# harmoniqs/Piccolo.jl

Hardware: AMD Instinct MI355X
Metric: constraint+Jacobian evals/sec, 3-transmon d=27 unitary, T=100 knots (higher is better)
Workload: dtype f64

## Files before the change

piccolo.jl_amd/csrc/pcl_device_common.hpp:

```cpp
#pragma once

#define PCL_DBG_WG 1024
#define PCL_DBG_WORDS (64 + 2 * PCL_DBG_WG)

#define PCL_NSP 8

typedef double double4_t __attribute__((ext_vector_type(4)));
typedef double double2_t __attribute__((ext_vector_type(2)));

struct KParams {
    const double *Z;
    const double *mu;
    double *delta;
    double *jac;
    double *hess;
    const double *G0;
    const int *upos;
    const double *ucoef;
    const int *csr_ptr;
    const int *csr_col;
    const double *csr_val;
    const int *csc_ptr;
    const int *csc_row;
    const double *csc_val;
    const int *x_offs;
    int x_off0;
    const int *umap;
    const double *ell_val;
    const int *ell_col;
    int ell_w, ell_lds;
    const unsigned char *uell_l;
    const double *uell_v;
    int uell_w;
    const double *ellt_val;
    const int *ellt_col;
    int ellt_w;
    const double *ug0;
    double *hpart;
    unsigned int *hcnt;
    int prof;
    long long *dbg;
    int ncw;
    int tab_lds;
    int contig;
    int all_matrix;
    int n_stream;
    int iso;
    long long z_batch_stride;
    long long g0_batch_stride;
    long long jac_per;
    long long hess_per;
    int n_upos;
    int d, n, m, K, z_dim, u_off, dt_off, batch;
    int cols;
    int nc;
    int S;
    int LD;
    int compact;
    int nt;
    double *expm;
    double *xout;
    int q;
    int lds_doubles;
    double pc[6];
    double *mpart;
    const double *mlam;
    int tail_mode;
    int v4_np;
    int v4_flags;
    unsigned int *tick;
    int tick_cpi;
    int tick_G;
    int tick_ahead;
    int *err;
};

template <bool TRANS_A>
__device__ __forceinline__ void mfma_gemm_lds(const double *__restrict__ A, int lda, const double *__restrict__ B,
                                              int ldb, double *__restrict__ C, int ldc, int M, int Nc, int Kd,
                                              int wave, int nwaves, int lane) {
    const int rt_n = (M + 15) >> 4, ct_n = (Nc + 15) >> 4, ks_n = (Kd + 3) >> 2;
    const int nt = rt_n * ct_n;
    const int li = lane & 15, lk = lane >> 4;
    for (int t0 = wave * 2; t0 < nt; t0 += nwaves * 2) {
        const int t1 = t0 + 1;
        const bool has1 = t1 < nt;
        const int rt0 = t0 % rt_n, ct0 = t0 / rt_n;
        const int rt1 = has1 ? t1 % rt_n : rt0, ct1 = has1 ? t1 / rt_n : ct0;
        const int row0 = rt0 * 16 + li, col0 = ct0 * 16 + li;
        const int row1 = rt1 * 16 + li, col1 = ct1 * 16 + li;
        const bool r0 = row0 < M, c0 = col0 < Nc, r1 = has1 && row1 < M, c1 = has1 && col1 < Nc;
        double4_t acc0 = {0.0, 0.0, 0.0, 0.0}, acc1 = {0.0, 0.0, 0.0, 0.0};
        for (int ks = 0; ks < ks_n; ++ks) {
            const int k = ks * 4 + lk;
            const bool kok = k < Kd;
            double a0 = 0.0, b0 = 0.0, a1 = 0.0, b1 = 0.0;
            if (r0 && kok) a0 = TRANS_A ? A[k + lda * row0] : A[row0 + lda * k];
            if (c0 && kok) b0 = B[k + ldb * col0];
            if (r1 && kok) a1 = TRANS_A ? A[k + lda * row1] : A[row1 + lda * k];
            if (c1 && kok) b1 = B[k + ldb * col1];
            acc0 = __builtin_amdgcn_mfma_f64_16x16x4f64(a0, b0, acc0, 0, 0, 0);
            acc1 = __builtin_amdgcn_mfma_f64_16x16x4f64(a1, b1, acc1, 0, 0, 0);
        }
        if (c0) {
#pragma unroll
            for (int r = 0; r < 4; ++r) {
                const int rr = rt0 * 16 + lk + 4 * r;
                if (rr < M) C[rr + ldc * col0] = acc0[r];
            }
        }
        if (c1) {
#pragma unroll
            for (int r = 0; r < 4; ++r) {
                const int rr = rt1 * 16 + lk + 4 * r;
                if (rr < M) C[rr + ldc * col1] = acc1[r];
            }
        }
    }
}

template <bool TRANS_A, bool ACC>
__device__ __forceinline__ void mfma_gemm_lds_acc(const double *__restrict__ A, int lda, const double *__restrict__ B, int ldb,
                                                  double *__restrict__ C, int ldc, int M, int Nc, int Kd, double alpha, int wave,
                                                  int nwaves, int lane) {
    const int rt_n = (M + 15) >> 4, ct_n = (Nc + 15) >> 4, ks_n = (Kd + 3) >> 2;
    const int nt = rt_n * ct_n;
    const int li = lane & 15, lk = lane >> 4;
    for (int t0 = wave * 2; t0 < nt; t0 += nwaves * 2) {
        const int t1 = t0 + 1;
        const bool has1 = t1 < nt;
        const int rt0 = t0 % rt_n, ct0 = t0 / rt_n;
        const int rt1 = has1 ? t1 % rt_n : rt0, ct1 = has1 ? t1 / rt_n : ct0;
        const int row0 = rt0 * 16 + li, col0 = ct0 * 16 + li;
        const int row1 = rt1 * 16 + li, col1 = ct1 * 16 + li;
        const bool r0 = row0 < M, c0 = col0 < Nc, r1 = has1 && row1 < M, c1 = has1 && col1 < Nc;
        double4_t acc0 = {0.0, 0.0, 0.0, 0.0}, acc1 = {0.0, 0.0, 0.0, 0.0};
        if (ACC) {
#pragma unroll
            for (int r = 0; r < 4; ++r) {
                const int rr0 = rt0 * 16 + lk + 4 * r, rr1 = rt1 * 16 + lk + 4 * r;
                if (c0 && rr0 < M) acc0[r] = C[rr0 + ldc * col0];
                if (c1 && rr1 < M) acc1[r] = C[rr1 + ldc * col1];
            }
        }
        for (int ks = 0; ks < ks_n; ks += 4) {
            double a0[4], b0[4], a1[4], b1[4];
#pragma unroll
            for (int u = 0; u < 4; ++u) {
                const int k = (ks + u) * 4 + lk;
                const bool kok = k < Kd;
                const bool pa0 = r0 && kok, pb0 = c0 && kok, pa1 = r1 && kok, pb1 = c1 && kok;
                const double va0 = A[pa0 ? (TRANS_A ? k + lda * row0 : row0 + lda * k) : 0], vb0 = B[pb0 ? k + ldb * col0 : 0];
                const double va1 = A[pa1 ? (TRANS_A ? k + lda * row1 : row1 + lda * k) : 0], vb1 = B[pb1 ? k + ldb * col1 : 0];
                a0[u] = pa0 ? alpha * va0 : 0.0;
                b0[u] = pb0 ? vb0 : 0.0;
                a1[u] = pa1 ? alpha * va1 : 0.0;
                b1[u] = pb1 ? vb1 : 0.0;
            }
#pragma unroll
            for (int u = 0; u < 4; ++u)
                if (ks + u < ks_n) {
                    acc0 = __builtin_amdgcn_mfma_f64_16x16x4f64(a0[u], b0[u], acc0, 0, 0, 0);
                    acc1 = __builtin_amdgcn_mfma_f64_16x16x4f64(a1[u], b1[u], acc1, 0, 0, 0);
                }
        }
        if (c0) {
#pragma unroll
            for (int r = 0; r < 4; ++r) {
                const int rr = rt0 * 16 + lk + 4 * r;
                if (rr < M) C[rr + ldc * col0] = acc0[r];
            }
        }
        if (c1) {
#pragma unroll
            for (int r = 0; r < 4; ++r) {
                const int rr = rt1 * 16 + lk + 4 * r;
                if (rr < M) C[rr + ldc * col1] = acc1[r];
            }
        }
    }
}
template <bool TRANS_A, bool ACC>
__device__ __forceinline__ void gemm_lds_acc(const double *A, int lda, const double *B, int ldb, double *C, int ldc, int M, int Nc, int Kd,
                                             double alpha) {
    mfma_gemm_lds_acc<TRANS_A, ACC>(A, lda, B, ldb, C, ldc, M, Nc, Kd, alpha, threadIdx.x >> 6, blockDim.x >> 6, threadIdx.x & 63);
}

template <bool TRANS_A>
__device__ __forceinline__ void valu_gemm_lds(const double *__restrict__ A, int lda, const double *__restrict__ B,
                                              int ldb, double *__restrict__ C, int ldc, int M, int Nc, int Kd,
                                              int tid, int nthreads) {
    for (int e = tid; e < M * Nc; e += nthreads) {
        const int i = e % M, j = e / M;
        double s = 0.0;
        for (int k = 0; k < Kd; ++k) s = fma(TRANS_A ? A[k + lda * i] : A[i + lda * k], B[k + ldb * j], s);
        C[i + ldc * j] = s;
    }
}

template <bool MFMA, bool TRANS_A>
__device__ __forceinline__ void gemm_lds(const double *A, int lda, const double *B, int ldb, double *C, int ldc, int M,
                                         int Nc, int Kd) {
    if (MFMA)
        mfma_gemm_lds<TRANS_A>(A, lda, B, ldb, C, ldc, M, Nc, Kd, threadIdx.x >> 6, blockDim.x >> 6,
                               threadIdx.x & 63);
    else
        valu_gemm_lds<TRANS_A>(A, lda, B, ldb, C, ldc, M, Nc, Kd, threadIdx.x, blockDim.x);
}

__device__ __forceinline__ void store2(double *p, double a, double b, int nt) {
    double2_t v = {a, b};
    if (nt == 2)
        asm volatile("global_store_dwordx4 %0, %1, off sc0 sc1" ::"v"(p), "v"(v) : "memory");
    else if (nt)
        __builtin_nontemporal_store(v, reinterpret_cast<double2_t *>(p));
    else
        *reinterpret_cast<double2_t *>(p) = v;
}

__device__ __forceinline__ void bpm_entry(double id, double c1, double c2, double g, double h2, double &mbp, double &bm) {
    const double e = __builtin_fma(c2, h2, id);
    mbp = -__builtin_fma(c1, g, e);
    bm = __builtin_fma(-c1, g, e);
}

template <int NT, bool TRANSPOSE = false>
__device__ __forceinline__ void load_tile(const double *__restrict__ src, double *__restrict__ dst, int n, int LD, int tid) {
    const int nn = n * n;
    for (int e0 = tid; e0 < nn; e0 += NT * 8) {
        double v[8];
#pragma unroll
        for (int j = 0; j < 8; ++j) v[j] = e0 + NT * j < nn ? src[e0 + NT * j] : 0.0;
#pragma unroll
        for (int j = 0; j < 8; ++j) {
            const int e = e0 + NT * j;
            if (e < nn) dst[TRANSPOSE ? (e / n) + LD * (e % n) : (e % n) + LD * (e / n)] = v[j];
        }
    }
}

__device__ __forceinline__ void build_G(const KParams &p, const double *__restrict__ G0, const double *__restrict__ zk,
                                        double *__restrict__ G, double *__restrict__ us) {
    const int n = p.n, LD = p.LD;
    for (int e = threadIdx.x; e < n * n; e += blockDim.x) G[(e % n) + LD * (e / n)] = G0[e];
    if ((int)threadIdx.x < p.m) us[threadIdx.x] = zk[p.u_off + threadIdx.x];
    __syncthreads();
    for (int q = threadIdx.x; q < p.n_upos; q += blockDim.x) {
        const int pos = p.upos[q];
        const int idx = (pos % n) + LD * (pos / n);
        double g = G[idx];
        for (int l = 0; l < p.m; ++l) g += us[l] * p.ucoef[(long long)q * p.m + l];
        G[idx] = g;
    }
}

__device__ __forceinline__ void wave_lds_sync() {
    asm volatile("s_waitcnt lgkmcnt(0)" ::: "memory");
    __builtin_amdgcn_wave_barrier();
}

#define PCL_MAXRT 4
#define PCL_MREG 8
#define PCL_PFC 4
#define PCL_PFW 2

__device__ __forceinline__ double wave_sum(double v) {
    for (int off = 32; off > 0; off >>= 1) v += __shfl_down(v, off, 64);
    return v;
}

template <int CTRL>
__device__ __forceinline__ double dpp_f64(double v) {
    int lo = __double2loint(v), hi = __double2hiint(v);
    lo = __builtin_amdgcn_update_dpp(lo, lo, CTRL, 0xf, 0xf, false);
    hi = __builtin_amdgcn_update_dpp(hi, hi, CTRL, 0xf, 0xf, false);
    return __hiloint2double(hi, lo);
}
__device__ __forceinline__ double row16_sum(double v) {
    v += dpp_f64<0xB1>(v);
    v += dpp_f64<0x4E>(v);
    v += dpp_f64<0x141>(v);
    v += dpp_f64<0x140>(v);
    return v;
}
```

piccolo.jl_amd/csrc/pcl_kernel_exp.hpp:

```cpp
#pragma once

#define PCL_EXP_COMPACT 1
#define PCL_EXP_MERIT 2

template <bool JAC, int MODE = 0>
__global__ __launch_bounds__(512) void pcl_exp_kernel(const KParams p, const double *__restrict__ Gjd, const int gl_lds) {
    extern __shared__ double lds[];
    constexpr bool COMPACT = JAC && (MODE & PCL_EXP_COMPACT), MERIT = JAC && (MODE & PCL_EXP_MERIT);
    const int n = p.n, LD = p.LD, nn = n * n, cols = p.cols;
    const int tid = threadIdx.x, nth = blockDim.x;
    const int ml = JAC ? max(p.m, 1) : 1;
    const int l = blockIdx.x % ml;
    const long long bk = blockIdx.x / ml;
    const int k = (int)(bk % p.K), b = (int)(bk / p.K);
    const bool fre = JAC && p.m > 0;
    const int tile = LD * n;
    double *A = lds, *T = A + tile, *S = T + tile;
    double *X = JAC ? S + tile : nullptr;
    double *Gl = (fre && gl_lds) ? X + tile : nullptr;
    double *XK = lds + ((JAC ? 4 : 3) + (Gl ? 1 : 0)) * tile;
    double *us = XK + LD * cols, *red = us + 32;
    const double *zk = p.Z + (long long)b * p.z_batch_stride + (long long)k * p.z_dim;
    const double *G0 = p.G0 + (long long)b * p.g0_batch_stride;
    const double *Gv = fre ? Gjd + (long long)l * nn : nullptr;
    const double h = zk[p.dt_off];
    build_G(p, G0, zk, A, us);
    __syncthreads();
    if (tid < 64) {
        double cs = 0.0;
        if (tid < n)
            for (int i = 0; i < n; ++i) cs += fabs(A[i + LD * tid]);
        red[tid] = cs;
    }
    __syncthreads();
    double nrm = 0.0;
    for (int j = 0; j < n; ++j) nrm = fmax(nrm, red[j]);
    double theta = fabs(h) * nrm;
    int sq = 0;
    while (theta > 0.25 && sq < 60) {
        theta *= 0.5;
        ++sq;
    }
    const double hs = ldexp(h, -sq);
    for (int e = tid; e < nn; e += nth) {
        const int idx = (e % n) + LD * (e / n);
        T[idx] = (e % n == e / n) ? 1.0 : 0.0;
        if (fre) X[idx] = 0.0;
        if (Gl) Gl[idx] = Gv[e];
    }
    __syncthreads();
    for (int j = 14; j >= 1; --j) {
        const double f = hs / j;
        if (fre) {
            gemm_lds<true, false>(A, LD, X, LD, S, LD, n, n, n);
            __syncthreads();
            if (Gl)
                gemm_lds<true, false>(Gl, LD, T, LD, X, LD, n, n, n);
            else
                gemm_lds<true, false>(Gv, n, T, LD, X, LD, n, n, n);
            __syncthreads();
            for (int e = tid; e < nn; e += nth) {
                const int idx = (e % n) + LD * (e / n);
                S[idx] = f * (S[idx] + X[idx]);
            }
            double *t = X;
            X = S;
            S = t;
            __syncthreads();
        }
        gemm_lds<true, false>(A, LD, T, LD, S, LD, n, n, n);
        __syncthreads();
        for (int e = tid; e < nn; e += nth) {
            const int idx = (e % n) + LD * (e / n);
            T[idx] = ((e % n == e / n) ? 1.0 : 0.0) + f * S[idx];
        }
        __syncthreads();
    }
    for (int i = 0; i < sq; ++i) {
        if (fre) {
            gemm_lds<true, false>(T, LD, X, LD, S, LD, n, n, n);
            gemm_lds<true, false>(X, LD, T, LD, A, LD, n, n, n);
            __syncthreads();
            for (int e = tid; e < nn; e += nth) {
                const int idx = (e % n) + LD * (e / n);
                X[idx] = S[idx] + A[idx];
            }
            __syncthreads();
        }
        gemm_lds<true, false>(T, LD, T, LD, S, LD, n, n, n);
        __syncthreads();
        double *t = T;
        T = S;
        S = t;
    }
    const int xo = p.x_off0 >= 0 ? p.x_off0 : p.x_offs[b];
    const int ne = n * cols;
    for (int e = tid; e < ne; e += nth) XK[(e % n) + LD * (e / n)] = zk[xo + e];
    __syncthreads();
    double *jv = JAC ? p.jac + bk * p.jac_per : nullptr;
    const int ncopy = COMPACT ? 1 : cols;
    const long long seg1 = (long long)ncopy * nn, tail0 = seg1 + (COMPACT ? 0 : ne);
    const int tw = (p.m + 1) * n;
    const double *lam = MERIT && p.mlam ? p.mlam + bk * ne : nullptr;
    double *part = MERIT ? p.mpart + bk * (p.m + 2) : nullptr;
    if (fre) {
        gemm_lds<true, false>(X, LD, XK, LD, S, LD, n, cols, n);
        if (MERIT && !lam) gemm_lds<true, false>(T, LD, XK, LD, A, LD, n, cols, n);
        __syncthreads();
        for (int e = tid; e < ne; e += nth) jv[tail0 + (long long)(e / n) * tw + l * n + (e % n)] = -S[(e % n) + LD * (e / n)];
        if (MERIT) {
            double v = 0.0;
            for (int e = tid; e < ne; e += nth) {
                const int idx = (e % n) + LD * (e / n);
                v = fma(lam ? lam[e] : zk[p.z_dim + xo + e] - A[idx], -S[idx], v);
            }
            v = exph_block_sum(v, red);
            if (tid == 0) part[l] = v;
        }
        __syncthreads();
    }
    if (l == 0) {
        gemm_lds<true, false>(T, LD, XK, LD, S, LD, n, cols, n);
        __syncthreads();
        if (p.delta) {
            double *dl = p.delta + bk * ne;
            for (int e = tid; e < ne; e += nth) dl[e] = zk[p.z_dim + xo + e] - S[(e % n) + LD * (e / n)];
        }
        if (JAC) {
            if (fre && (sq > 0 || (MERIT && !lam))) {
                build_G(p, G0, zk, A, us);
                __syncthreads();
            }
            gemm_lds<true, false>(A, LD, S, LD, X, LD, n, cols, n);
            __syncthreads();
            for (int e = tid; e < ne; e += nth) {
                jv[tail0 + (long long)(e / n) * tw + p.m * n + (e % n)] = -X[(e % n) + LD * (e / n)];
                if (!COMPACT) jv[seg1 + e] = 1.0;
            }
            if (MERIT) {
                double vh = 0.0, vp = 0.0;
                for (int e = tid; e < ne; e += nth) {
                    const int idx = (e % n) + LD * (e / n);
                    const double dl = zk[p.z_dim + xo + e] - S[idx], lm = lam ? lam[e] : dl;
                    vh = fma(lm, -X[idx], vh);
                    vp = fma(lm, dl, vp);
                }
                vh = exph_block_sum(vh, red);
                vp = exph_block_sum(vp, red);
                if (tid == 0) {
                    part[p.m] = vh;
                    part[p.m + 1] = lam ? vp : 0.5 * vp;
                }
            }
        }
    }
    if (JAC) {
        if (!(n & 1) && !((unsigned long long)jv & 15ull)) {
            const int half = nn >> 1;
            for (int c = l; c < ncopy; c += ml) {
                double *dst = jv + (long long)c * nn;
                for (int e2 = tid; e2 < half; e2 += nth) {
                    const int e = 2 * e2, idx = (e % n) + LD * (e / n);
                    const double2_t v = {-T[idx], -T[idx + 1]};
                    *reinterpret_cast<double2_t *>(dst + e) = v;
                }
            }
        } else {
            for (int c = l; c < ncopy; c += ml) {
                double *dst = jv + (long long)c * nn;
                for (int e = tid; e < nn; e += nth) dst[e] = -T[(e % n) + LD * (e / n)];
            }
        }
    }
}
```

Before: 40960.

## Restructure MFMA f64 GEMM tiles with double-buffered loads and shared operand pairs

Replaces both MFMA LDS GEMM paths with one templated tile-pair routine. It double-buffers operand loads (P/Q slots with sched_barrier) so LDS reads overlap MFMA issue, and reuses the A or B fragment when the two tiles a wave handles share a row or column block. It also peels the K tail out of the main loop and removes per-iteration bounds predicates. Separately, the elementwise loops in the expm kernel now step row and column indices incrementally instead of computing e%n and e/n each iteration. This adds code complexity and template instantiations, and may raise register pressure.

```diff
diff --git a/piccolo.jl_amd/csrc/pcl_device_common.hpp b/piccolo.jl_amd/csrc/pcl_device_common.hpp
--- a/piccolo.jl_amd/csrc/pcl_device_common.hpp
+++ b/piccolo.jl_amd/csrc/pcl_device_common.hpp
@@ -75,110 +75,169 @@
     int *err;
 };
 
-template <bool TRANS_A>
+#ifndef PCL_GEMM_U
+#define PCL_GEMM_U 1
+#endif
+enum { PCL_PAIR_GENERAL = 0, PCL_PAIR_SHARED_B = 1, PCL_PAIR_SHARED_A = 2, PCL_PAIR_SINGLE = 3 };
+
+template <bool TRANS_A, bool ACC, bool SCALED, int U, int MODE>
+__device__ __forceinline__ void mfma_tile_pair(const double *__restrict__ A, int lda, const double *__restrict__ B, int ldb,
+                                               double *__restrict__ C, int ldc, int M, int Nc, int Kd, double alpha, int rt0, int ct0,
+                                               int rt1, int ct1, int li, int lk) {
+    constexpr bool PAIR = MODE != PCL_PAIR_SINGLE;
+    constexpr bool A1 = MODE == PCL_PAIR_GENERAL || MODE == PCL_PAIR_SHARED_B;
+    constexpr bool B1 = MODE == PCL_PAIR_GENERAL || MODE == PCL_PAIR_SHARED_A;
+    const int row0 = rt0 * 16 + li, col0 = ct0 * 16 + li, row1 = rt1 * 16 + li, col1 = ct1 * 16 + li;
+    const bool c0 = col0 < Nc, c1 = PAIR && col1 < Nc;
+    const int rc0 = row0 < M ? row0 : 0, cc0 = c0 ? col0 : 0, rc1 = row1 < M ? row1 : 0, cc1 = c1 ? col1 : 0;
+    const int oa0 = TRANS_A ? lk + lda * rc0 : rc0 + lda * lk, oa1 = TRANS_A ? lk + lda * rc1 : rc1 + lda * lk;
+    const int ob0 = lk + ldb * cc0, ob1 = lk + ldb * cc1;
+    const int sa = TRANS_A ? 4 : 4 * lda;
+    const int ks_full = Kd >> 2;
+    double4_t acc0 = {0.0, 0.0, 0.0, 0.0}, acc1 = {0.0, 0.0, 0.0, 0.0};
+    struct Slots {
+        double a0[U], b0[U], a1[U], b1[U];
+    } P, Q;
+    auto load = [&](Slots &s, int u, int ks) {
+        const double va0 = A[oa0 + sa * ks];
+        s.a0[u] = SCALED ? alpha * va0 : va0;
+        s.b0[u] = B[ob0 + 4 * ks];
+        if (A1) {
+            const double va1 = A[oa1 + sa * ks];
+            s.a1[u] = SCALED ? alpha * va1 : va1;
+        }
+        if (B1) s.b1[u] = B[ob1 + 4 * ks];
+    };
+    auto product = [&](double x0, double y0, double x1, double y1) {
+        acc0 = __builtin_amdgcn_mfma_f64_16x16x4f64(x0, y0, acc0, 0, 0, 0);
+        if (PAIR) acc1 = __builtin_amdgcn_mfma_f64_16x16x4f64(A1 ? x1 : x0, B1 ? y1 : y0, acc1, 0, 0, 0);
+    };
+    const bool tail = (Kd & 3) != 0;
+    double ta0 = 0.0, tb0 = 0.0, ta1 = 0.0, tb1 = 0.0;
+    if (tail) {
+        const bool kok = ks_full * 4 + lk < Kd;
+        const double va0 = A[kok ? oa0 + sa * ks_full : 0], vb0 = B[kok ? ob0 + 4 * ks_full : 0];
+        ta0 = kok ? (SCALED ? alpha * va0 : va0) : 0.0;
+        tb0 = kok ? vb0 : 0.0;
+        if (A1) {
+            const double va1 = A[kok ? oa1 + sa * ks_full : 0];
+            ta1 = kok ? (SCALED ? alpha * va1 : va1) : 0.0;
+        }
+        if (B1) {
+            const double vb1 = B[kok ? ob1 + 4 * ks_full : 0];
+            tb1 = kok ? vb1 : 0.0;
+        }
+    }
+    if (ACC) {
+#pragma unroll
+        for (int r = 0; r < 4; ++r) {
+            const int rr0 = rt0 * 16 + lk + 4 * r, rr1 = rt1 * 16 + lk + 4 * r;
+            if (c0 && rr0 < M) acc0[r] = C[rr0 + ldc * col0];
+            if (c1 && rr1 < M) acc1[r] = C[rr1 + ldc * col1];
+        }
+    }
+    auto request_whole = [&](Slots &s, int ks) {
+#pragma unroll
+        for (int u = 0; u < U; ++u) load(s, u, ks + u);
+    };
+    auto request = [&](Slots &s, int ks) {
+#pragma unroll
+        for (int u = 0; u < U; ++u) load(s, u, ks + u < ks_full ? ks + u : ks_full - 1);
+    };
+    auto spend_whole = [&](const Slots &s) {
+#pragma unroll
+        for (int u = 0; u < U; ++u) product(s.a0[u], s.b0[u], s.a1[u], s.b1[u]);
+    };
+    auto spend = [&](const Slots &s, int nb) {
+        if (nb >= U) {
+            spend_whole(s);
+        } else {
+#pragma unroll
+            for (int u = 0; u < U; ++u)
+                if (u < nb) product(s.a0[u], s.b0[u], s.a1[u], s.b1[u]);
+        }
+    };
+    if (ks_full > 0) {
+        int ks = 0;
+        request(P, 0);
+        for (; ks + 3 * U <= ks_full; ks += 2 * U) {
+            request_whole(Q, ks + U);
+            __builtin_amdgcn_sched_barrier(0x6);
+            spend_whole(P);
+            __builtin_amdgcn_sched_barrier(0x6);
+            request_whole(P, ks + 2 * U);
+            __builtin_amdgcn_sched_barrier(0x6);
+            spend_whole(Q);
+            __builtin_amdgcn_sched_barrier(0x6);
+        }
+        const int left = ks_full - ks;
+        if (left > U) request(Q, ks + U);
+        __builtin_amdgcn_sched_barrier(0x6);
+        spend(P, left);
+        if (left > U) {
+            __builtin_amdgcn_sched_barrier(0x6);
+            if (left > 2 * U) request(P, ks + 2 * U);
+            __builtin_amdgcn_sched_barrier(0x6);
+            spend(Q, left - U);
+            if (left > 2 * U) spend(P, left - 2 * U);
+        }
+    }
+    if (tail) product(ta0, tb0, ta1, tb1);
+    if (c0) {
+#pragma unroll
+        for (int r = 0; r < 4; ++r) {
+            const int rr = rt0 * 16 + lk + 4 * r;
+            if (rr < M) C[rr + ldc * col0] = acc0[r];
+        }
+    }
+    if (c1) {
+#pragma unroll
+        for (int r = 0; r < 4; ++r) {
+            const int rr = rt1 * 16 + lk + 4 * r;
+            if (rr < M) C[rr + ldc * col1] = acc1[r];
+        }
+    }
+}
+
+template <bool TRANS_A, bool ACC, bool SCALED, int U>
+__device__ __forceinline__ void mfma_gemm_tiles(const double *__restrict__ A, int lda, const double *__restrict__ B, int ldb,
+                                                double *__restrict__ C, int ldc, int M, int Nc, int Kd, double alpha, int wave,
+                                                int nwaves, int lane) {
+    const int rt_n = (M + 15) >> 4, ct_n = (Nc + 15) >> 4;
+    const int li = lane & 15, lk = lane >> 4;
+    const int step = 2 * nwaves;
+    int rt0 = 2 * __builtin_amdgcn_readfirstlane(wave), ct0 = 0;
+    if (rt_n <= 0) return;
+    for (;; rt0 += step) {
+        while (rt0 >= rt_n) rt0 -= rt_n, ++ct0;
+        if (ct0 >= ct_n) break;
+        const bool wrap = rt0 + 1 == rt_n;
+        const int rt1 = wrap ? 0 : rt0 + 1, ct1 = wrap ? ct0 + 1 : ct0;
+#define PCL_TILE_PAIR(MODE) mfma_tile_pair<TRANS_A, ACC, SCALED, U, MODE>(A, lda, B, ldb, C, ldc, M, Nc, Kd, alpha, rt0, ct0, rt1, ct1, li, lk)
+        if (ct1 >= ct_n)
+            PCL_TILE_PAIR(PCL_PAIR_SINGLE);
+        else if (!wrap)
+            PCL_TILE_PAIR(PCL_PAIR_SHARED_B);
+        else if (rt_n == 1)
+            PCL_TILE_PAIR(PCL_PAIR_SHARED_A);
+        else
+            mfma_tile_pair<TRANS_A, ACC, SCALED, (U > 1 ? U / 2 : 1), PCL_PAIR_GENERAL>(A, lda, B, ldb, C, ldc, M, Nc, Kd, alpha, rt0, ct0, rt1, ct1, li, lk);
+#undef PCL_TILE_PAIR
+    }
+}
+
+template <bool TRANS_A, int U = PCL_GEMM_U>
 __device__ __forceinline__ void mfma_gemm_lds(const double *__restrict__ A, int lda, const double *__restrict__ B,
                                               int ldb, double *__restrict__ C, int ldc, int M, int Nc, int Kd,
                                               int wave, int nwaves, int lane) {
-    const int rt_n = (M + 15) >> 4, ct_n = (Nc + 15) >> 4, ks_n = (Kd + 3) >> 2;
-    const int nt = rt_n * ct_n;
-    const int li = lane & 15, lk = lane >> 4;
-    for (int t0 = wave * 2; t0 < nt; t0 += nwaves * 2) {
-        const int t1 = t0 + 1;
-        const bool has1 = t1 < nt;
-        const int rt0 = t0 % rt_n, ct0 = t0 / rt_n;
-        const int rt1 = has1 ? t1 % rt_n : rt0, ct1 = has1 ? t1 / rt_n : ct0;
-        const int row0 = rt0 * 16 + li, col0 = ct0 * 16 + li;
-        const int row1 = rt1 * 16 + li, col1 = ct1 * 16 + li;
-        const bool r0 = row0 < M, c0 = col0 < Nc, r1 = has1 && row1 < M, c1 = has1 && col1 < Nc;
-        double4_t acc0 = {0.0, 0.0, 0.0, 0.0}, acc1 = {0.0, 0.0, 0.0, 0.0};
-        for (int ks = 0; ks < ks_n; ++ks) {
-            const int k = ks * 4 + lk;
-            const bool kok = k < Kd;
-            double a0 = 0.0, b0 = 0.0, a1 = 0.0, b1 = 0.0;
-            if (r0 && kok) a0 = TRANS_A ? A[k + lda * row0] : A[row0 + lda * k];
-            if (c0 && kok) b0 = B[k + ldb * col0];
-            if (r1 && kok) a1 = TRANS_A ? A[k + lda * row1] : A[row1 + lda * k];
-            if (c1 && kok) b1 = B[k + ldb * col1];
-            acc0 = __builtin_amdgcn_mfma_f64_16x16x4f64(a0, b0, acc0, 0, 0, 0);
-            acc1 = __builtin_amdgcn_mfma_f64_16x16x4f64(a1, b1, acc1, 0, 0, 0);
-        }
-        if (c0) {
-#pragma unroll
-            for (int r = 0; r < 4; ++r) {
-                const int rr = rt0 * 16 + lk + 4 * r;
-                if (rr < M) C[rr + ldc * col0] = acc0[r];
-            }
-        }
-        if (c1) {
-#pragma unroll
-            for (int r = 0; r < 4; ++r) {
-                const int rr = rt1 * 16 + lk + 4 * r;
-                if (rr < M) C[rr + ldc * col1] = acc1[r];
-            }
-        }
-    }
-}
-
-template <bool TRANS_A, bool ACC>
+    mfma_gemm_tiles<TRANS_A, false, false, U>(A, lda, B, ldb, C, ldc, M, Nc, Kd, 1.0, wave, nwaves, lane);
+}
+
+template <bool TRANS_A, bool ACC, int U = PCL_GEMM_U>
 __device__ __forceinline__ void mfma_gemm_lds_acc(const double *__restrict__ A, int lda, const double *__restrict__ B, int ldb,
                                                   double *__restrict__ C, int ldc, int M, int Nc, int Kd, double alpha, int wave,
                                                   int nwaves, int lane) {
-    const int rt_n = (M + 15) >> 4, ct_n = (Nc + 15) >> 4, ks_n = (Kd + 3) >> 2;
-    const int nt = rt_n * ct_n;
-    const int li = lane & 15, lk = lane >> 4;
-    for (int t0 = wave * 2; t0 < nt; t0 += nwaves * 2) {
-        const int t1 = t0 + 1;
-        const bool has1 = t1 < nt;
-        const int rt0 = t0 % rt_n, ct0 = t0 / rt_n;
-        const int rt1 = has1 ? t1 % rt_n : rt0, ct1 = has1 ? t1 / rt_n : ct0;
-        const int row0 = rt0 * 16 + li, col0 = ct0 * 16 + li;
-        const int row1 = rt1 * 16 + li, col1 = ct1 * 16 + li;
-        const bool r0 = row0 < M, c0 = col0 < Nc, r1 = has1 && row1 < M, c1 = has1 && col1 < Nc;
-        double4_t acc0 = {0.0, 0.0, 0.0, 0.0}, acc1 = {0.0, 0.0, 0.0, 0.0};
-        if (ACC) {
-#pragma unroll
-            for (int r = 0; r < 4; ++r) {
-                const int rr0 = rt0 * 16 + lk + 4 * r, rr1 = rt1 * 16 + lk + 4 * r;
-                if (c0 && rr0 < M) acc0[r] = C[rr0 + ldc * col0];
-                if (c1 && rr1 < M) acc1[r] = C[rr1 + ldc * col1];
-            }
-        }
-        for (int ks = 0; ks < ks_n; ks += 4) {
-            double a0[4], b0[4], a1[4], b1[4];
-#pragma unroll
-            for (int u = 0; u < 4; ++u) {
-                const int k = (ks + u) * 4 + lk;
-                const bool kok = k < Kd;
-                const bool pa0 = r0 && kok, pb0 = c0 && kok, pa1 = r1 && kok, pb1 = c1 && kok;
-                const double va0 = A[pa0 ? (TRANS_A ? k + lda * row0 : row0 + lda * k) : 0], vb0 = B[pb0 ? k + ldb * col0 : 0];
-                const double va1 = A[pa1 ? (TRANS_A ? k + lda * row1 : row1 + lda * k) : 0], vb1 = B[pb1 ? k + ldb * col1 : 0];
-                a0[u] = pa0 ? alpha * va0 : 0.0;
-                b0[u] = pb0 ? vb0 : 0.0;
-                a1[u] = pa1 ? alpha * va1 : 0.0;
-                b1[u] = pb1 ? vb1 : 0.0;
-            }
-#pragma unroll
-            for (int u = 0; u < 4; ++u)
-                if (ks + u < ks_n) {
-                    acc0 = __builtin_amdgcn_mfma_f64_16x16x4f64(a0[u], b0[u], acc0, 0, 0, 0);
-                    acc1 = __builtin_amdgcn_mfma_f64_16x16x4f64(a1[u], b1[u], acc1, 0, 0, 0);
-                }
-        }
-        if (c0) {
-#pragma unroll
-            for (int r = 0; r < 4; ++r) {
-                const int rr = rt0 * 16 + lk + 4 * r;
-                if (rr < M) C[rr + ldc * col0] = acc0[r];
-            }
-        }
-        if (c1) {
-#pragma unroll
-            for (int r = 0; r < 4; ++r) {
-                const int rr = rt1 * 16 + lk + 4 * r;
-                if (rr < M) C[rr + ldc * col1] = acc1[r];
-            }
-        }
-    }
+    mfma_gemm_tiles<TRANS_A, ACC, true, U>(A, lda, B, ldb, C, ldc, M, Nc, Kd, alpha, wave, nwaves, lane);
 }
 template <bool TRANS_A, bool ACC>
 __device__ __forceinline__ void gemm_lds_acc(const double *A, int lda, const double *B, int ldb, double *C, int ldc, int M, int Nc, int Kd,
@@ -207,6 +266,19 @@
     else
         valu_gemm_lds<TRANS_A>(A, lda, B, ldb, C, ldc, M, Nc, Kd, threadIdx.x, blockDim.x);
 }
+
+struct TileWalkStart {
+    int n, e0, r0, c0, de, dr, dc;
+    __device__ __forceinline__ TileWalkStart(int n_, int tid, int nth) : n(n_), e0(tid), r0(tid % n_), c0(tid / n_), de(nth), dr(nth % n_), dc(nth / n_) {}
+};
+struct TileWalk {
+    int e, r, c;
+    __device__ __forceinline__ explicit TileWalk(const TileWalkStart &s) : e(s.e0), r(s.r0), c(s.c0) {}
+    __device__ __forceinline__ void next(const TileWalkStart &s) {
+        e += s.de, r += s.dr, c += s.dc;
+        if (r >= s.n) r -= s.n, ++c;
+    }
+};
 
 __device__ __forceinline__ void store2(double *p, double a, double b, int nt) {
     double2_t v = {a, b};
diff --git a/piccolo.jl_amd/csrc/pcl_kernel_exp.hpp b/piccolo.jl_amd/csrc/pcl_kernel_exp.hpp
--- a/piccolo.jl_amd/csrc/pcl_kernel_exp.hpp
+++ b/piccolo.jl_amd/csrc/pcl_kernel_exp.hpp
@@ -42,6 +42,7 @@
         ++sq;
     }
     const double hs = ldexp(h, -sq);
+    const TileWalkStart wk(n, tid, nth);
     for (int e = tid; e < nn; e += nth) {
         const int idx = (e % n) + LD * (e / n);
         T[idx] = (e % n == e / n) ? 1.0 : 0.0;
@@ -59,8 +60,8 @@
             else
                 gemm_lds<true, false>(Gv, n, T, LD, X, LD, n, n, n);
             __syncthreads();
-            for (int e = tid; e < nn; e += nth) {
-                const int idx = (e % n) + LD * (e / n);
+            for (TileWalk w(wk); w.e < nn; w.next(wk)) {
+                const int idx = w.r + LD * w.c;
                 S[idx] = f * (S[idx] + X[idx]);
             }
             double *t = X;
@@ -70,9 +71,9 @@
         }
         gemm_lds<true, false>(A, LD, T, LD, S, LD, n, n, n);
         __syncthreads();
-        for (int e = tid; e < nn; e += nth) {
-            const int idx = (e % n) + LD * (e / n);
-            T[idx] = ((e % n == e / n) ? 1.0 : 0.0) + f * S[idx];
+        for (TileWalk w(wk); w.e < nn; w.next(wk)) {
+            const int idx = w.r + LD * w.c;
+            T[idx] = ((w.r == w.c) ? 1.0 : 0.0) + f * S[idx];
         }
         __syncthreads();
     }
@@ -81,8 +82,8 @@
             gemm_lds<true, false>(T, LD, X, LD, S, LD, n, n, n);
             gemm_lds<true, false>(X, LD, T, LD, A, LD, n, n, n);
             __syncthreads();
-            for (int e = tid; e < nn; e += nth) {
-                const int idx = (e % n) + LD * (e / n);
+            for (TileWalk w(wk); w.e < nn; w.next(wk)) {
+                const int idx = w.r + LD * w.c;
                 X[idx] = S[idx] + A[idx];
             }
             __syncthreads();
```

Result: no change. 41080 (median of 3 runs) (+0.3%).
